# google/compare_gan

Hardware: NVIDIA H100
Metric: images/sec G+D step (resnet_cifar10) (higher is better)
Workload: dtype tf32

## Files before the change

### compare_gan_b200/_lib.py

```python
import ctypes
import os
import re

HERE = os.path.dirname(os.path.abspath(__file__))
HEADER = os.path.join(HERE, "..", "include", "cgan_b200.h")
SO_PATH = os.path.join(HERE, "csrc", "libcgan_b200.so")


class ConvDesc(ctypes.Structure):
  _fields_ = [(n, ctypes.c_int32) for n in
              ("n", "h", "w", "cin", "cout", "kh", "kw", "stride", "upsample", "oh", "ow", "pad_t", "pad_l")]


class ConvEpilogue(ctypes.Structure):
  _fields_ = [("bias", ctypes.c_void_p), ("residual", ctypes.c_void_p), ("mask", ctypes.c_void_p),
              ("mask_leak", ctypes.c_float), ("flags", ctypes.c_int32), ("ldy", ctypes.c_int32)]


CONV_RELU, CONV_ROUND_OUT, CONV_IN_TF32, CONV_IN2_TF32 = 1, 2, 4, 8
ACT_ROUND_TF32 = 0x100
OPT_TC_MT, OPT_LAST_PATH, OPT_TC_HALO, OPT_TC_THIN = 1, 2, 3, 6
OPT_LAST_TC_BN, OPT_LAST_TC_MT, OPT_LAST_TC_HALO, OPT_LAST_TC_CTAS_PER_SM = 7, 8, 9, 10
PATH_NAMES = {0: "simt_fp32", 1: "tcgen05_tf32", 2: "thin_fp32"}

_SCALARS = {"int": ctypes.c_int, "int32_t": ctypes.c_int32, "int64_t": ctypes.c_int64,
            "float": ctypes.c_float, "double": ctypes.c_double, "size_t": ctypes.c_size_t, "uint64_t": ctypes.c_uint64}


def parse_header(path=HEADER):
  src = open(path).read()
  src = re.sub(r"/\*.*?\*/", " ", src, flags=re.S)
  src = re.sub(r"//[^\n]*", " ", src)
  protos = {}
  for m in re.finditer(r"(const\s+char\s*\*|int64_t|int)\s+(cgan_\w+)\s*\(([^;{]*)\)\s*;", src):
    ret, name, args = m.group(1), m.group(2), m.group(3)
    restype = ctypes.c_char_p if "char" in ret else (ctypes.c_int64 if ret == "int64_t" else ctypes.c_int)
    argtypes = []
    args = args.strip()
    if args and args != "void":
      for a in args.split(","):
        a = a.strip()
        if "*" in a:
          argtypes.append(ctypes.c_void_p)
        else:
          ty = a.replace("const", "").split()[0]
          argtypes.append(_SCALARS[ty])
    protos[name] = (restype, argtypes)
  return protos


class CganError(RuntimeError):
  pass


_DLL = {}
# ... 65 lines not shown
```

### compare_gan_b200/csrc/common.cuh

```cuda
#pragma once
#include <cuda_runtime.h>
#include <stdint.h>
#include <stdio.h>
#include <string.h>

#include "../../include/cgan_b200.h"

struct cgan_ctx {
  int device;
  cudaStream_t stream;
  void* ws;
  size_t ws_bytes;
  int math_mode;
  int64_t launches;
  int num_sms;
  int tc_mt_max;
  int tc_halo;
  int tc_thin;
  int last_path;
  int last_tc_bn, last_tc_mt, last_tc_halo;
  int last_tc_ctas_per_sm;
  unsigned* counters;
  void* p2p;
  char err[512];
};

constexpr int CGAN_NUM_COUNTERS = 1 << 18;

static inline int cgan_fail(cgan_ctx* ctx, int code, const char* fmt, const char* a = "", const char* b = "") {
  if (ctx) snprintf(ctx->err, sizeof(ctx->err), fmt, a, b);
  return code;
}

#define CGAN_REQUIRE(ctx, cond, msg)                                              \
  do {                                                                            \
    if (!(cond)) return cgan_fail((ctx), CGAN_ERR_ARG, "%s: %s", __func__, msg);  \
  } while (0)

#define CGAN_CUDA(ctx, call)                                                                        \
  do {                                                                                              \
    cudaError_t e__ = (call);                                                                       \
    if (e__ != cudaSuccess) return cgan_fail((ctx), CGAN_ERR_CUDA, "%s: %s", __func__, cudaGetErrorString(e__)); \
  } while (0)

#define CGAN_LAUNCHED(ctx)                                                                          \
  do {                                                                                              \
    (ctx)->launches++;                                                                              \
    cudaError_t e__ = cudaGetLastError();                                                           \
    if (e__ != cudaSuccess) return cgan_fail((ctx), CGAN_ERR_CUDA, "%s: launch: %s", __func__, cudaGetErrorString(e__)); \
  } while (0)

static inline int cgan_ws(cgan_ctx* ctx, size_t bytes, void** out) {
  if (bytes > ctx->ws_bytes) {
    cudaStreamCaptureStatus st = cudaStreamCaptureStatusNone;
// ... 218 lines not shown
```

### compare_gan_b200/csrc/conv_tc.cu

```cuda
#include "tc_common.cuh"

namespace {

using namespace tc;

constexpr int TC_BM = 128;
constexpr int TC_BK = 32;
constexpr int TC_MAX_STAGES = 4;
constexpr int TC_MAX_TAPS = 32;
constexpr int TC_CWARPS = 8;
constexpr int TC_THREADS = 32 * TC_CWARPS + 32;
constexpr int TC_A_BYTES = TC_BM * TC_BK * 4;
constexpr int TC_WG_A_BYTES = TC_A_BYTES / 2;
constexpr int TC_ACC_COLS = 256;

struct TcParams {
  int ntaps, kchunks;
  int off_h[TC_MAX_TAPS], off_w[TC_MAX_TAPS], wtap[TC_MAX_TAPS], amap[TC_MAX_TAPS];
  int bw, bh, bni;
  int tiles_w, tiles_h;
  int rows_used;
  int img_n, img_h, img_w;
  int relu;
  int vec2;
  int round_a;
  int round_out;
  float mask_leak;
  const float* residual;
  const float* mask;
  int wimg_stride;
  int bn;
  int stages;
  int mt;
  int tiles_total;
  int cout;
  long long s_n, s_h, s_w, base;
  float* out;
  const float* bias;
  int nphases;
  int ph_tap0[5];
  long long ph_base[4];
  int hg, hnv;
  int h_off_w[4], h_off_h0[4], h_wtap[4][4];
  int a_halo_bytes;
  int a_box_bytes;
  int sa_stages, sb_stages;
};

struct AMaps { CUtensorMap m[4]; };


__device__ __forceinline__ void tc_tile_origin(const TcParams& p, int t, int& ow0, int& oh0, int& n0) {
  const int tw = t % p.tiles_w; t /= p.tiles_w;
  const int th = t % p.tiles_h;
  const int tn = t / p.tiles_h;
  ow0 = tw * p.bw; oh0 = th * p.bh; n0 = tn * p.bni;
}

__device__ __forceinline__ float epilogue_one(const TcParams& p, float v, int col, long long off) {
  if (p.bias) v += p.bias[col];
  if (p.residual) v += p.residual[off];
  if (p.relu) v = fmaxf(v, 0.f);
  if (p.mask) v = p.mask[off] > 0.f ? v : p.mask_leak * v;
  if (p.round_out) v = rna_tf32(v);
  return v;
}

template <int BN>
__device__ __forceinline__ void tile_epilogue(const TcParams& p, const float* acc, int tile, int nb0, int wg, int warp, int lane,
                                            long long out_base) {
  int ow0, oh0, n0;
  tc_tile_origin(p, tile, ow0, oh0, n0);
  const int c2 = (lane & 3) * 2;
#pragma unroll
  for (int h = 0; h < 2; ++h) {
    const int m = wg * 64 + (warp & 3) * 16 + (lane >> 2) + h * 8;
    const int wi = m % p.bw;
    const int hi = (m / p.bw) % p.bh;
    const int ni = m / (p.bw * p.bh);
    if (!(m < p.rows_used && n0 + ni < p.img_n && oh0 + hi < p.img_h && ow0 + wi < p.img_w)) continue;
    const long long roff = out_base + (long long)(n0 + ni) * p.s_n + (long long)(oh0 + hi) * p.s_h +
                           (long long)(ow0 + wi) * p.s_w + nb0;
#pragma unroll
    for (int j = 0; j < BN / 8; ++j) {
      const int c = j * 8 + c2;
      if (nb0 + c >= p.cout) continue;
      float2 v = make_float2(acc[4 * j + 2 * h], acc[4 * j + 2 * h + 1]);
      const long long off = roff + c;
      if (p.vec2) {
        if (p.bias) { const float2 b = *reinterpret_cast<const float2*>(p.bias + nb0 + c); v.x += b.x; v.y += b.y; }
        if (p.residual) { const float2 r = *reinterpret_cast<const float2*>(p.residual + off); v.x += r.x; v.y += r.y; }
        if (p.relu) { v.x = fmaxf(v.x, 0.f); v.y = fmaxf(v.y, 0.f); }
        if (p.mask) {
          const float2 mv = *reinterpret_cast<const float2*>(p.mask + off);
          v.x = mv.x > 0.f ? v.x : p.mask_leak * v.x; v.y = mv.y > 0.f ? v.y : p.mask_leak * v.y;
        }
        if (p.round_out) { v.x = rna_tf32(v.x); v.y = rna_tf32(v.y); }
        *reinterpret_cast<float2*>(p.out + off) = v;
      } else {
        p.out[off] = epilogue_one(p, v.x, nb0 + c, off);
        if (nb0 + c + 1 < p.cout) p.out[off + 1] = epilogue_one(p, v.y, nb0 + c + 1, off + 1);
      }
    }
  }
}

constexpr int tc_min_ctas(int bn, int mt) { return bn * mt <= 128 ? 2 : 1; }

__device__ __forceinline__ void tc_round_smem(uint32_t base, int bytes, int q, int nthreads) {
#pragma unroll 4
  for (int i = q * 16; i < bytes; i += nthreads * 16) {
    float4 v = lds128(base + i);
    v.x = rna_tf32(v.x); v.y = rna_tf32(v.y); v.z = rna_tf32(v.z); v.w = rna_tf32(v.w);
    sts128(base + i, v);
  }
}

template <int BN, int MT>
__global__ void __launch_bounds__(TC_THREADS, tc_min_ctas(BN, MT))
conv_tc_kernel(const __grid_constant__ AMaps tm_as, const __grid_constant__ CUtensorMap tm_b, const TcParams p) {
  extern __shared__ __align__(1024) uint8_t smem_raw[];
  uint8_t* smem = reinterpret_cast<uint8_t*>((reinterpret_cast<uintptr_t>(smem_raw) + 1023) & ~uintptr_t(1023));
  constexpr int b_bytes = BN * TC_BK * 4;
  constexpr int a_bytes = MT * TC_A_BYTES;
  constexpr int stage_bytes = a_bytes + b_bytes;
  uint64_t* full_bar = reinterpret_cast<uint64_t*>(smem + p.stages * stage_bytes);
  uint64_t* empty_bar = full_bar + p.stages;

  const int warp = threadIdx.x >> 5, lane = threadIdx.x & 31;
  const int tap0 = p.ph_tap0[blockIdx.z];
  const int num_kb = (p.ph_tap0[blockIdx.z + 1] - tap0) * p.kchunks;

  const int tile0 = blockIdx.x * MT;
  const int nt_here = max(0, min(MT, p.tiles_total - tile0));
  const int nb0 = blockIdx.y * BN;

  if (threadIdx.x == 0) {
    for (int s = 0; s < p.stages; ++s) {
      mbar_init(&full_bar[s], 1);
      mbar_init(&empty_bar[s], 2);
    }
    asm volatile("fence.mbarrier_init.release.cluster;" ::: "memory");
  }
  __syncthreads();

  if (warp == TC_CWARPS) {
    if (lane == 0) {
      asm volatile("prefetch.tensormap [%0];" ::"l"(&tm_as.m[0]) : "memory");
      asm volatile("prefetch.tensormap [%0];" ::"l"(&tm_b) : "memory");
      int stage = 0;
      uint32_t phase = 0;
      for (int kb = 0; kb < num_kb; ++kb) {
        const int tl = kb / p.kchunks, kc = kb - tl * p.kchunks, tap = tap0 + tl;
        mbar_wait(&empty_bar[stage], phase ^ 1);
        uint8_t* sa = smem + stage * stage_bytes;
        uint8_t* sb = sa + a_bytes;
        mbar_expect_tx(&full_bar[stage], (uint32_t)(nt_here * p.rows_used * TC_BK * 4 + b_bytes));
        int ow0, oh0, n0;
        for (int i = 0; i < nt_here; ++i) {
          tc_tile_origin(p, tile0 + i, ow0, oh0, n0);
          tma_load_4d(sa + i * TC_A_BYTES, &tm_as.m[p.amap[tap]], &full_bar[stage], kc * TC_BK, ow0 + p.off_w[tap],
                      oh0 + p.off_h[tap], n0);
        }
        tc_tile_origin(p, tile0, ow0, oh0, n0);
        tma_load_3d(sb, &tm_b, &full_bar[stage], kc * TC_BK, nb0, p.wtap[tap] + n0 * p.wimg_stride);
        if (++stage == p.stages) { stage = 0; phase ^= 1; }
      }
    }
  } else {
    const int wg = warp >> 2;
    const int q = threadIdx.x & 127;
    float acc[MT][BN / 2];
#pragma unroll
    for (int t = 0; t < MT; ++t)
#pragma unroll
      for (int i = 0; i < BN / 2; ++i) acc[t][i] = 0.f;
    int stage = 0, prev = -1;
    uint32_t phase = 0;
    for (int kb = 0; kb < num_kb; ++kb) {
      mbar_wait(&full_bar[stage], phase);
      const uint32_t a_addr = smem_u32(smem + stage * stage_bytes) + wg * TC_WG_A_BYTES;
      const uint32_t b_addr = smem_u32(smem + stage * stage_bytes) + a_bytes;
      if (p.round_a) {
        for (int tl = 0; tl < nt_here; ++tl) tc_round_smem(a_addr + tl * TC_A_BYTES, TC_WG_A_BYTES, q, 128);
        fence_proxy_async();
        named_bar(1 + wg, 128);
      }
#pragma unroll
      for (int t = 0; t < MT; ++t)
#pragma unroll
        for (int i = 0; i < BN / 2; ++i) acc_fence(acc[t][i]);
      wgmma_fence();
#pragma unroll
      for (int t = 0; t < MT; ++t) {
#pragma unroll
        for (int k = 0; k < TC_BK / 8; ++k)
          wgmma_tf32<BN>(acc[t], make_desc(a_addr + t * TC_A_BYTES + k * 32), make_desc(b_addr + k * 32));
      }
      wgmma_commit();
      wgmma_wait<1>();
#pragma unroll
      for (int t = 0; t < MT; ++t)
#pragma unroll
        for (int i = 0; i < BN / 2; ++i) acc_fence(acc[t][i]);
      if (prev >= 0 && q == 0) mbar_arrive(&empty_bar[prev]);
      prev = stage;
      if (++stage == p.stages) { stage = 0; phase ^= 1; }
    }
    wgmma_wait<0>();
#pragma unroll
    for (int t = 0; t < MT; ++t) {
#pragma unroll
      for (int i = 0; i < BN / 2; ++i) acc_fence(acc[t][i]);
      if (t < nt_here) tile_epilogue<BN>(p, acc[t], tile0 + t, nb0, wg, warp, lane, p.ph_base[blockIdx.z]);
    }
  }
}

template <int BN, int MT>
__global__ void __launch_bounds__(TC_THREADS, 1)
conv_tc_halo_kernel(const __grid_constant__ CUtensorMap tm_a, const __grid_constant__ CUtensorMap tm_b, const TcParams p) {
  extern __shared__ __align__(1024) uint8_t smem_raw[];
  uint8_t* smem = reinterpret_cast<uint8_t*>((reinterpret_cast<uintptr_t>(smem_raw) + 1023) & ~uintptr_t(1023));
  constexpr int b_bytes = BN * TC_BK * 4;
  const int a_stage = MT * p.a_halo_bytes;
  uint8_t* smem_b = smem + p.sa_stages * a_stage;
  uint64_t* a_full = reinterpret_cast<uint64_t*>(smem_b + p.sb_stages * b_bytes);
  uint64_t* a_empty = a_full + p.sa_stages;
  uint64_t* b_full = a_empty + p.sa_stages;
  uint64_t* b_empty = b_full + p.sb_stages;

  const int warp = threadIdx.x >> 5, lane = threadIdx.x & 31;
  const int tile0 = blockIdx.x * MT;
  const int nt_here = min(MT, p.tiles_total - tile0);
  const int nb0 = blockIdx.y * BN;

  if (threadIdx.x == 0) {
    for (int s = 0; s < p.sa_stages; ++s) {
      mbar_init(&a_full[s], 1);
      mbar_init(&a_empty[s], 2);
    }
    for (int s = 0; s < p.sb_stages; ++s) {
      mbar_init(&b_full[s], 1);
      mbar_init(&b_empty[s], 2);
    }
    asm volatile("fence.mbarrier_init.release.cluster;" ::: "memory");
  }
// ... 125 lines not shown
  int best = tc_pick_bn(ncols_pad);
  if (best == 0 || tiles_m * (ncols_pad / best) >= sms) return best;
  int pick = best;
  for (int b = best - 32; b >= 64; b -= 32) {
    if (ncols_pad % b) continue;
    pick = b;
    if (tiles_m * (ncols_pad / b) >= sms) break;
  }
  return pick;
}

constexpr int TC_NARROW_WAVES = 2;
constexpr int TC_NARROW_MAX_KB = 96;

inline int tc_pick_bn_per_tap(int ncols_pad, long long tiles_m, const TcParams& p, int sms) {
  const int bn = tc_pick_bn_occupancy(ncols_pad, tiles_m, sms);
  int kb = 0;
  for (int i = 0; i < p.nphases; ++i) {
    const int k = (p.ph_tap0[i + 1] - p.ph_tap0[i]) * p.kchunks;
    if (k > kb) kb = k;
  }
  if (bn == 256 && tiles_m * (ncols_pad / 256) * p.nphases >= (long long)TC_NARROW_WAVES * sms && kb <= TC_NARROW_MAX_KB)
    return 128;
  return bn;
}


inline int tc_vec2(const TcParams& p) {
  long long odd = p.cout | p.s_n | p.s_h | p.s_w | p.base;
  for (int i = 0; i < p.nphases; ++i) odd |= p.ph_base[i];
  return (odd & 1) ? 0 : 1;
}

int prep_weights(cgan_ctx* ctx, const TcConv& c, int kdim_pad, int ncols_pad, float** out) {
  void* ws = nullptr;
  int rc = cgan_ws(ctx, (size_t)c.taps_total * ncols_pad * kdim_pad * sizeof(float), &ws);
  if (rc) return rc;
  float* wt = reinterpret_cast<float*>(ws);
  long long tot = (long long)c.taps_total * ncols_pad * kdim_pad;
  long long blocks = (tot + 255) / 256, cap = (long long)ctx->num_sms * 8;
  wprep_kernel<<<(int)(blocks > cap ? cap : blocks), 256, 0, ctx->stream>>>(wt, c.wsrc, c.taps_total, c.ncols, ncols_pad, c.a.ch,
                                                                             kdim_pad, c.transpose_w);
  CGAN_LAUNCHED(ctx);
  *out = wt;
  return CGAN_OK;
}

bool make_weight_map(CUtensorMap* tm, float* wt, int kdim_pad, int ncols_pad, int taps_total, int bn) {
  cuuint64_t dims[3] = {(cuuint64_t)kdim_pad, (cuuint64_t)ncols_pad, (cuuint64_t)taps_total};
  cuuint64_t strides[2] = {(cuuint64_t)kdim_pad * 4, (cuuint64_t)ncols_pad * kdim_pad * 4};
  cuuint32_t box[3] = {TC_BK, (cuuint32_t)bn, 1};
  cuuint32_t es[3] = {1, 1, 1};
  return get_encode()(tm, CU_TENSOR_MAP_DATA_TYPE_FLOAT32, 3, wt, dims, strides, box, es, CU_TENSOR_MAP_INTERLEAVE_NONE,
                      CU_TENSOR_MAP_SWIZZLE_128B, CU_TENSOR_MAP_L2_PROMOTION_L2_256B,
                      CU_TENSOR_MAP_FLOAT_OOB_FILL_NONE) == CUDA_SUCCESS;
}

template <typename Kernel>
int tc_ctas_per_sm(Kernel kernel, size_t smem) {
  int blocks = 0;
  if (cudaOccupancyMaxActiveBlocksPerMultiprocessor(&blocks, kernel, TC_THREADS, smem) != cudaSuccess) blocks = 0;
  return blocks;
}

template <int BN, int MT>
int tc_launch_t(cgan_ctx* ctx, bool halo, dim3 grid, size_t smem, const AMaps& as, const CUtensorMap& b, const TcParams& p) {
  static bool attr_set[2] = {false, false};
  if (halo) {
    if (!attr_set[1]) {
      CGAN_CUDA(ctx, cudaFuncSetAttribute(conv_tc_halo_kernel<BN, MT>, cudaFuncAttributeMaxDynamicSharedMemorySize, 227 * 1024));
      attr_set[1] = true;
    }
    ctx->last_tc_ctas_per_sm = tc_ctas_per_sm(conv_tc_halo_kernel<BN, MT>, smem);
    conv_tc_halo_kernel<BN, MT><<<grid, TC_THREADS, smem, ctx->stream>>>(as.m[0], b, p);
  } else {
    if (!attr_set[0]) {
      CGAN_CUDA(ctx, cudaFuncSetAttribute(conv_tc_kernel<BN, MT>, cudaFuncAttributeMaxDynamicSharedMemorySize, 227 * 1024));
      attr_set[0] = true;
    }
    ctx->last_tc_ctas_per_sm = tc_ctas_per_sm(conv_tc_kernel<BN, MT>, smem);
    conv_tc_kernel<BN, MT><<<grid, TC_THREADS, smem, ctx->stream>>>(as, b, p);
  }
  CGAN_LAUNCHED(ctx);
  return CGAN_OK;
}

int tc_launch(cgan_ctx* ctx, bool halo, dim3 grid, size_t smem, const AMaps& as, const CUtensorMap& b, const TcParams& p) {
  ctx->last_tc_bn = p.bn; ctx->last_tc_mt = p.mt; ctx->last_tc_halo = halo ? 1 : 0;
#define TC_CASE(BN, MT) \
  if (p.bn == BN && p.mt == MT) return tc_launch_t<BN, MT>(ctx, halo, grid, smem, as, b, p);
  TC_CASE(32, 1) TC_CASE(64, 1) TC_CASE(96, 1) TC_CASE(128, 1) TC_CASE(160, 1) TC_CASE(192, 1) TC_CASE(224, 1)
  TC_CASE(256, 1) TC_CASE(32, 2) TC_CASE(64, 2) TC_CASE(96, 2) TC_CASE(128, 2)
#undef TC_CASE
  return cgan_fail(ctx, CGAN_ERR_UNSUPPORTED, "%s: no kernel for this column tile / pixel-tile count%s", "cgan_conv_tc");
}

}

bool cgan_tc_shape_ok(int n, int h, int w, int kdim, int ncols) {
  if (n < 1 || h < 1 || w < 1 || ncols < 1) return false;
  if (kdim < 8 || kdim % 4 != 0) return false;
  if (ncols > 256 && ncols % 32 != 0) return false;
  int bn = tc_pick_bn((ncols + 31) / 32 * 32);
  return bn != 0 && bn % 32 == 0;
}

int cgan_conv_tc(cgan_ctx* ctx, const TcConv& c) {
  if (!get_encode()) return cgan_fail(ctx, CGAN_ERR_UNSUPPORTED, "%s: cuTensorMapEncodeTiled unavailable%s", "cgan_conv_tc");
  const ConvTaps& tp = c.taps;
  if (tp.ntaps > TC_MAX_TAPS || c.a.nviews > 4) return cgan_fail(ctx, CGAN_ERR_UNSUPPORTED, "%s: too many taps/views%s", "cgan_conv_tc");
  const int n = c.a.n, h = c.a.h, w = c.a.w, kdim = c.a.ch, gh = c.gh, gw = c.gw, ntaps = tp.ntaps;
  TcParams p;
  memset(&p, 0, sizeof(p));
  p.ntaps = ntaps;
  const int kdim_pad = (kdim + TC_BK - 1) / TC_BK * TC_BK;
  p.kchunks = kdim_pad / TC_BK;
  for (int i = 0; i < ntaps; ++i) {
    p.off_h[i] = tp.off_h[i]; p.off_w[i] = tp.off_w[i]; p.wtap[i] = tp.wtap[i]; p.amap[i] = tp.view[i];
  }
  int tiles_n;
  tc_geometry(n, gh, gw, &p.bw, &p.bh, &p.bni, &p.tiles_w, &p.tiles_h, &tiles_n);
  p.rows_used = p.bw * p.bh * p.bni;
  p.img_n = n; p.img_h = gh; p.img_w = gw;
// ... 59 lines not shown
      p.tiles_w = w / hbw; p.tiles_h = h / hbh;
      const long long tiles_total = (long long)p.tiles_w * p.tiles_h * n;
      p.rows_used = 128;
      p.bn = tc_pick_bn_occupancy(ncols_pad, tiles_total, ctx->num_sms);
      const int ncol_tiles = ncols_pad / p.bn;
      p.a_box_bytes = (hbh + 2) * hbw * 128;
      p.a_halo_bytes = (p.a_box_bytes + 1023) / 1024 * 1024;
      const int b_bytes = p.bn * TC_BK * 4;
      const int budget = 227 * 1024 - 1024 - 512;
      const int mt_cap = ctx->tc_mt_max >= 2 ? 2 : 1;
      p.sa_stages = 2;
      p.mt = 1;
      for (int m = mt_cap; m >= 2; --m) {
        if (m * p.bn > TC_ACC_COLS || tiles_total * ncol_tiles < 2ll * m * ctx->num_sms) continue;
        if ((budget - p.sa_stages * m * p.a_halo_bytes) / b_bytes < 4) continue;
        p.mt = m;
        break;
      }
      p.sb_stages = (budget - p.sa_stages * p.mt * p.a_halo_bytes) / b_bytes;
      if (p.sb_stages > 8) p.sb_stages = 8;
      ok = p.sb_stages >= 2;
      if (ok) {
        p.tiles_total = (int)tiles_total;
        AMaps tm_a;
        CUtensorMap tm_b;
        memset(&tm_a, 0, sizeof(tm_a));
        if (!make_act_map(&tm_a.m[0], c.a.in + c.a.view_off[0], kdim, w, h, n, c.a.sw, c.a.sh, c.a.sn, hbw, hbh + 2, 1))
          return cgan_fail(ctx, CGAN_ERR_CUDA, "%s: cuTensorMapEncodeTiled(A halo) failed%s", "cgan_conv_tc");
        if (!make_weight_map(&tm_b, wt, kdim_pad, ncols_pad, c.taps_total, p.bn))
          return cgan_fail(ctx, CGAN_ERR_CUDA, "%s: cuTensorMapEncodeTiled(B) failed%s", "cgan_conv_tc");
        p.vec2 = tc_vec2(p);
        size_t smem = (size_t)p.sa_stages * p.mt * p.a_halo_bytes + (size_t)p.sb_stages * b_bytes + 1024 + 512;
        dim3 grid((unsigned)((tiles_total + p.mt - 1) / p.mt), (unsigned)ncol_tiles);
        return tc_launch(ctx, true, grid, smem, tm_a, tm_b, p);
      }
    }
    tc_geometry(n, gh, gw, &p.bw, &p.bh, &p.bni, &p.tiles_w, &p.tiles_h, &tiles_n);
    p.rows_used = p.bw * p.bh * p.bni;
    p.bn = tc_pick_bn_per_tap(ncols_pad, (long long)p.tiles_w * p.tiles_h * tiles_n, p, ctx->num_sms);
    p.hg = p.hnv = 0;
  }

  AMaps tm_as;
  CUtensorMap tm_b;
  memset(&tm_as, 0, sizeof(tm_as));
  for (int v = 0; v < 4; ++v)
    if (!make_view_map(&tm_as.m[v], c.a, v, p.bw, p.bh, p.bni))
      return cgan_fail(ctx, CGAN_ERR_CUDA, "%s: cuTensorMapEncodeTiled(A) failed%s", "cgan_conv_tc");
  if (!make_weight_map(&tm_b, wt, kdim_pad, ncols_pad, c.taps_total, p.bn))
    return cgan_fail(ctx, CGAN_ERR_CUDA, "%s: cuTensorMapEncodeTiled(B) failed%s", "cgan_conv_tc");

  const long long tiles_total = (long long)p.tiles_w * p.tiles_h * tiles_n;
  const int ncol_tiles = ncols_pad / p.bn;
  p.tiles_total = (int)tiles_total;
  p.mt = 1;
  if (ctx->tc_mt_max >= 2 && 2 * p.bn <= 128 && tiles_total * ncol_tiles * p.nphases >= 4ll * ctx->num_sms &&
      (c.wimg_stride == 0 || (p.tiles_w * p.tiles_h) % 2 == 0))
    p.mt = 2;
  const bool two_ctas = p.mt * p.bn <= 128;
  const size_t stage_bytes = (size_t)p.mt * TC_A_BYTES + (size_t)p.bn * TC_BK * 4;
  p.stages = (int)(((two_ctas ? 110 : 220) * 1024) / stage_bytes);
  if (p.stages > TC_MAX_STAGES) p.stages = TC_MAX_STAGES;
  if (p.stages < 2) p.stages = 2;
  p.vec2 = tc_vec2(p);
  size_t smem = (size_t)p.stages * stage_bytes + 1024  + 256 ;
  dim3 grid((unsigned)((tiles_total + p.mt - 1) / p.mt), (unsigned)ncol_tiles, (unsigned)p.nphases);
  return tc_launch(ctx, false, grid, smem, tm_as, tm_b, p);
}
```

### compare_gan_b200/csrc/pointwise.cu

```cuda
#include "common.cuh"

int cgan_version(void) { return 1; }

int cgan_ctx_create(cgan_ctx** out, int device) {
  if (!out) return CGAN_ERR_ARG;
  *out = nullptr;
  int count = 0;
  if (cudaGetDeviceCount(&count) != cudaSuccess || device < 0 || device >= count) return CGAN_ERR_CUDA;
  cgan_ctx* c = new cgan_ctx();
  memset(c, 0, sizeof(*c));
  c->device = device;
  if (cudaSetDevice(device) != cudaSuccess) { delete c; return CGAN_ERR_CUDA; }
  cudaDeviceProp prop;
  if (cudaGetDeviceProperties(&prop, device) != cudaSuccess) { delete c; return CGAN_ERR_CUDA; }
  c->num_sms = prop.multiProcessorCount;
  c->tc_mt_max = 2;
  if (const char* e = getenv("CGAN_TC_MT")) c->tc_mt_max = atoi(e) >= 2 ? 2 : 1;
  c->tc_halo = 1;
  if (const char* e = getenv("CGAN_TC_HALO")) c->tc_halo = atoi(e) ? 1 : 0;
  c->tc_thin = 1;
  if (const char* e = getenv("CGAN_TC_THIN")) c->tc_thin = atoi(e) ? 1 : 0;
  c->stream = 0;
  if (cudaMalloc(reinterpret_cast<void**>(&c->counters), CGAN_NUM_COUNTERS * sizeof(unsigned)) != cudaSuccess ||
      cudaMemset(c->counters, 0, CGAN_NUM_COUNTERS * sizeof(unsigned)) != cudaSuccess) {
// ... 33 lines not shown

int cgan_ctx_set_option(cgan_ctx* ctx, int key, int64_t value) {
  if (!ctx) return CGAN_ERR_ARG;
  switch (key) {
    case CGAN_OPT_TC_MT:
      CGAN_REQUIRE(ctx, value == 1 || value == 2, "CGAN_OPT_TC_MT must be 1 or 2");
      ctx->tc_mt_max = (int)value;
      return CGAN_OK;
    case CGAN_OPT_TC_HALO:
      CGAN_REQUIRE(ctx, value >= 0 && value <= 2, "CGAN_OPT_TC_HALO must be 0, 1 or 2");
      ctx->tc_halo = (int)value;
      return CGAN_OK;
    case CGAN_OPT_TC_THIN:
      CGAN_REQUIRE(ctx, value == 0 || value == 1, "CGAN_OPT_TC_THIN must be 0 or 1");
      ctx->tc_thin = (int)value;
      return CGAN_OK;
    default:
      return cgan_fail(ctx, CGAN_ERR_ARG, "%s: unknown or read-only option%s", "cgan_ctx_set_option");
  }
}

int cgan_ctx_get_option(cgan_ctx* ctx, int key, int64_t* host_value) {
  if (!ctx) return CGAN_ERR_ARG;
  CGAN_REQUIRE(ctx, host_value, "null pointer");
  switch (key) {
    case CGAN_OPT_TC_MT: *host_value = ctx->tc_mt_max; return CGAN_OK;
    case CGAN_OPT_LAST_PATH: *host_value = ctx->last_path; return CGAN_OK;
    case CGAN_OPT_TC_HALO: *host_value = ctx->tc_halo; return CGAN_OK;
    case CGAN_OPT_TC_THIN: *host_value = ctx->tc_thin; return CGAN_OK;
    case CGAN_OPT_LAST_TC_BN: *host_value = ctx->last_tc_bn; return CGAN_OK;
    case CGAN_OPT_LAST_TC_MT: *host_value = ctx->last_tc_mt; return CGAN_OK;
    case CGAN_OPT_LAST_TC_HALO: *host_value = ctx->last_tc_halo; return CGAN_OK;
    case CGAN_OPT_LAST_TC_CTAS_PER_SM: *host_value = ctx->last_tc_ctas_per_sm; return CGAN_OK;
    default:
      return cgan_fail(ctx, CGAN_ERR_ARG, "%s: unknown option%s", "cgan_ctx_get_option");
  }
}

const char* cgan_last_error(cgan_ctx* ctx) { return ctx ? ctx->err : "null context"; }
int64_t cgan_launch_count(cgan_ctx* ctx) { return ctx ? ctx->launches : -1; }

namespace {

#define EW_LOOP(i, n)                                                                  \
  for (long long i = (long long)blockIdx.x * blockDim.x + threadIdx.x, s__ = (long long)gridDim.x * blockDim.x; \
       i < (n); i += s__)

__global__ void fill_kernel(float* d, float v, long long n) { EW_LOOP(i, n) d[i] = v; }
__global__ void copy_kernel(float* __restrict__ d, const float* __restrict__ s, long long n) { EW_LOOP(i, n) d[i] = s[i]; }
__global__ void copy2d_kernel(float* __restrict__ d, int dld, int doff, const float* __restrict__ s, int sld, int soff,
                              long long rows, int cols) {
  long long n = rows * cols;
  EW_LOOP(i, n) {
    long long r = i / cols;
    int j = (int)(i % cols);
    d[r * dld + doff + j] = s[r * sld + soff + j];
  }
}
__global__ void axpby_kernel(float* __restrict__ y, float a, const float* __restrict__ x, float b,
                             const float* __restrict__ y0, float c, long long n) {
  EW_LOOP(i, n) {
    float v = a * x[i] + c;
    if (y0) v += b * y0[i];
    y[i] = v;
  }
}
// ... 810 lines not shown
```

### compare_gan_b200/csrc/tc_common.cuh

```cuda
#pragma once
#include <cuda.h>

#include "common.cuh"
#include "wgmma_tf32.cuh"

namespace tc {

__device__ __forceinline__ uint32_t smem_u32(const void* p) { return (uint32_t)__cvta_generic_to_shared(p); }

__device__ __forceinline__ void mbar_init(uint64_t* bar, uint32_t count) {
  asm volatile("mbarrier.init.shared::cta.b64 [%0], %1;" ::"r"(smem_u32(bar)), "r"(count));
}
__device__ __forceinline__ void mbar_expect_tx(uint64_t* bar, uint32_t bytes) {
  asm volatile("mbarrier.arrive.expect_tx.shared::cta.b64 _, [%0], %1;" ::"r"(smem_u32(bar)), "r"(bytes) : "memory");
}
__device__ __forceinline__ void mbar_arrive(uint64_t* bar) {
  asm volatile("mbarrier.arrive.shared::cta.b64 _, [%0];" ::"r"(smem_u32(bar)) : "memory");
}
__device__ __forceinline__ void mbar_wait(uint64_t* bar, uint32_t parity) {
  uint32_t addr = smem_u32(bar);
  asm volatile(
      "{\n\t"
      ".reg .pred p;\n\t"
      "WAIT_LOOP:\n\t"
// ... 11 lines not shown
}
__device__ __forceinline__ void tma_load_3d(void* dst, const CUtensorMap* map, uint64_t* bar, int c0, int c1, int c2) {
  asm volatile(
      "cp.async.bulk.tensor.3d.shared::cluster.global.tile.mbarrier::complete_tx::bytes [%0], [%1, {%3, %4, %5}], [%2];"
      ::"r"(smem_u32(dst)), "l"(map), "r"(smem_u32(bar)), "r"(c0), "r"(c1), "r"(c2) : "memory");
}

__device__ __forceinline__ uint64_t make_desc(uint32_t smem_addr) {
  uint64_t d = 0;
  d |= (uint64_t)((smem_addr & 0x3FFFF) >> 4);
  d |= (uint64_t)1 << 16;
  d |= (uint64_t)(1024 >> 4) << 32;
  d |= (uint64_t)1 << 62;
  return d;
}

__device__ __forceinline__ void wgmma_fence() { asm volatile("wgmma.fence.sync.aligned;" ::: "memory"); }
__device__ __forceinline__ void wgmma_commit() { asm volatile("wgmma.commit_group.sync.aligned;" ::: "memory"); }
template <int N>
__device__ __forceinline__ void wgmma_wait() { asm volatile("wgmma.wait_group.sync.aligned %0;" ::"n"(N) : "memory"); }
__device__ __forceinline__ void acc_fence(float& r) { asm volatile("" : "+f"(r)::"memory"); }
__device__ __forceinline__ void named_bar(int id, int count) { asm volatile("bar.sync %0, %1;" ::"r"(id), "r"(count) : "memory"); }
__device__ __forceinline__ void fence_proxy_async() { asm volatile("fence.proxy.async.shared::cta;" ::: "memory"); }

__device__ __forceinline__ uint32_t sw128_offset(int row, int k) {
  return (uint32_t)(row * 128 + ((((k >> 2) ^ row) & 7) << 4) + (k & 3) * 4);
}

__device__ __forceinline__ float4 lds128(uint32_t addr) {
  float4 v;
  asm volatile("ld.shared.v4.f32 {%0, %1, %2, %3}, [%4];" : "=f"(v.x), "=f"(v.y), "=f"(v.z), "=f"(v.w) : "r"(addr));
  return v;
}
__device__ __forceinline__ float lds32(uint32_t addr) {
  float v;
  asm volatile("ld.shared.f32 %0, [%1];" : "=f"(v) : "r"(addr));
  return v;
}
__device__ __forceinline__ void sts128(uint32_t addr, float4 v) {
  asm volatile("st.shared.v4.f32 [%0], {%1, %2, %3, %4};" ::"r"(addr), "f"(v.x), "f"(v.y), "f"(v.z), "f"(v.w) : "memory");
}

typedef CUresult (*EncodeTiledFn)(CUtensorMap*, CUtensorMapDataType, cuuint32_t, void*, const cuuint64_t*, const cuuint64_t*,
                                  const cuuint32_t*, const cuuint32_t*, CUtensorMapInterleave, CUtensorMapSwizzle,
                                  CUtensorMapL2promotion, CUtensorMapFloatOOBfill);

inline EncodeTiledFn get_encode() {
  static EncodeTiledFn fn = nullptr;
  if (!fn) {
    void* p = nullptr;
    cudaDriverEntryPointQueryResult q;
    if (cudaGetDriverEntryPoint("cuTensorMapEncodeTiled", &p, cudaEnableDefault, &q) == cudaSuccess &&
        q == cudaDriverEntryPointSuccess)
      fn = reinterpret_cast<EncodeTiledFn>(p);
  }
  return fn;
}


inline bool make_act_map(CUtensorMap* tm, const float* base, int c, int w, int h, int n, long long sw, long long sh,
                         long long sn, int bw, int bh, int bni, CUtensorMapSwizzle swizzle = CU_TENSOR_MAP_SWIZZLE_128B) {
  EncodeTiledFn enc = get_encode();
  if (!enc) return false;
  cuuint64_t dims[4] = {(cuuint64_t)c, (cuuint64_t)w, (cuuint64_t)h, (cuuint64_t)n};
  cuuint64_t strides[3] = {(cuuint64_t)sw * 4, (cuuint64_t)sh * 4, (cuuint64_t)sn * 4};
  cuuint32_t box[4] = {32, (cuuint32_t)bw, (cuuint32_t)bh, (cuuint32_t)bni};
// ... 17 lines not shown
```

### include/cgan_b200.h

```cpp
#ifndef CGAN_B200_H_
#define CGAN_B200_H_

#include <stddef.h>
#include <stdint.h>

#ifdef __cplusplus
extern "C" {
#endif

typedef struct cgan_ctx cgan_ctx;

enum { CGAN_OK = 0, CGAN_ERR_ARG = 1, CGAN_ERR_CUDA = 2, CGAN_ERR_WORKSPACE = 3, CGAN_ERR_UNSUPPORTED = 4 };

int cgan_version(void);
int cgan_ctx_create(cgan_ctx** out, int device);
int cgan_ctx_destroy(cgan_ctx* ctx);
int cgan_ctx_set_stream(cgan_ctx* ctx, void* cuda_stream);
int cgan_ctx_reserve_workspace(cgan_ctx* ctx, size_t bytes);
int cgan_ctx_set_math_mode(cgan_ctx* ctx, int mode);
const char* cgan_last_error(cgan_ctx* ctx);
int64_t cgan_launch_count(cgan_ctx* ctx);
enum { CGAN_OPT_TC_MT = 1, CGAN_OPT_LAST_PATH = 2, CGAN_OPT_TC_HALO = 3, CGAN_OPT_TC_THIN = 6, CGAN_OPT_LAST_TC_BN = 7,
       CGAN_OPT_LAST_TC_MT = 8, CGAN_OPT_LAST_TC_HALO = 9, CGAN_OPT_LAST_TC_CTAS_PER_SM = 10 };
enum { CGAN_PATH_SIMT_FP32 = 0, CGAN_PATH_TCGEN05_TF32 = 1, CGAN_PATH_THIN_FP32 = 2 };
int cgan_ctx_set_option(cgan_ctx* ctx, int key, int64_t value);
int cgan_ctx_get_option(cgan_ctx* ctx, int key, int64_t* host_value);

int cgan_fill(cgan_ctx*, float* dst, float value, int64_t n);
int cgan_copy(cgan_ctx*, float* dst, const float* src, int64_t n);
int cgan_copy2d(cgan_ctx*, float* dst, int dst_ld, int dst_off, const float* src, int src_ld, int src_off,
                int64_t rows, int cols);
int cgan_axpby(cgan_ctx*, float* y, float a, const float* x, float b, const float* y0, float c, int64_t n);
int cgan_scale_by_dev(cgan_ctx*, float* y, const float* x, const float* scalar_dev, float mul, int inverse, int64_t n);
int cgan_dot(cgan_ctx*, float* out_dev, const float* a, const float* b, int64_t n);
int cgan_random_uniform(cgan_ctx*, float* out, int64_t n, uint64_t seed, uint64_t offset);
int cgan_interpolate(cgan_ctx*, float* y, const float* x, const float* xf, const float* alpha, int n, int64_t per);
int cgan_one_hot(cgan_ctx*, float* out, const int32_t* labels, int n, int classes);

typedef struct {
  int32_t n, h, w, cin;
  int32_t cout, kh, kw, stride;
  int32_t upsample;
  int32_t oh, ow;
  int32_t pad_t, pad_l;
} cgan_conv_desc;

int cgan_conv2d_fwd(cgan_ctx*, const cgan_conv_desc*, const float* x, const float* w_hwio, const float* bias, float* y);
int cgan_conv2d_fwd_act(cgan_ctx*, const cgan_conv_desc*, const float* x, const float* w_hwio, const float* bias, int act,
                        float* y);
int cgan_conv2d_fwd_act_ld(cgan_ctx*, const cgan_conv_desc*, const float* x, const float* w_hwio, const float* bias, int act,
                           float* y, int ldy);
int cgan_conv2d_dgrad(cgan_ctx*, const cgan_conv_desc*, const float* dy, const float* w_hwio, float* dx);
int cgan_conv2d_wgrad(cgan_ctx*, const cgan_conv_desc*, const float* x, const float* dy, float* dw);
enum { CGAN_CONV_RELU = 1, CGAN_CONV_ROUND_OUT = 2, CGAN_CONV_IN_TF32 = 4, CGAN_CONV_IN2_TF32 = 8 };
typedef struct {
  const float* bias;
// ... 149 lines not shown
```

### profiles/tile_ab.py

```python
import argparse
import hashlib
import json
import os
import statistics
import subprocess
import sys

TF32_PEAK_TFLOPS = 495.0

SHAPES = [
    ("cifar G up 3x3 256->256 4->8", 256, 4, 256, 256, 3, True),
    ("cifar G up 3x3 256->256 8->16", 256, 8, 256, 256, 3, True),
    ("cifar G up 3x3 256->256 16->32", 256, 16, 256, 256, 3, True),
    ("cifar G 3x3 256->256 @8", 256, 8, 256, 256, 3, False),
    ("cifar G 3x3 256->256 @16", 256, 16, 256, 256, 3, False),
    ("cifar G 3x3 256->256 @32", 256, 32, 256, 256, 3, False),
    ("cifar G up 1x1 256->256 4->8", 256, 4, 256, 256, 1, True),
    ("cifar G up 1x1 256->256 8->16", 256, 8, 256, 256, 1, True),
    ("cifar G up 1x1 256->256 16->32", 256, 16, 256, 256, 1, True),
    ("cifar D 3x3 128->128 @32", 512, 32, 128, 128, 3, False),
    ("cifar D 1x1 128->128 @32", 512, 32, 128, 128, 1, False),
    ("cifar D 3x3 128->128 @16", 512, 16, 128, 128, 3, False),
    ("cifar D 3x3 128->128 @8", 512, 8, 128, 128, 3, False),
    ("biggan G up 3x3 1536->1536 4->8", 64, 4, 1536, 1536, 3, True),
# ... 23 lines not shown
    torch.cuda.synchronize()
    st = torch.cuda.current_stream()
    e0, e1 = torch.cuda.Event(enable_timing=True), torch.cuda.Event(enable_timing=True)
    e0.record(st)
    for _ in range(iters):
      fn()
    e1.record(st)
    torch.cuda.synchronize()
    return e0.elapsed_time(e1) / iters

  def rand(*shape):
    return K.from_numpy((np.random.RandomState(sum(shape)).standard_normal(shape) * 0.1).astype(np.float32))

  K.init(0)
  K.set_math_mode(1)
  lib = K.lib()
  ctas_key = getattr(_lib, "OPT_LAST_TC_CTAS_PER_SM", None)

  def digest(t):
    return hashlib.sha1(np.ascontiguousarray(t.cpu()).tobytes()).hexdigest()[:12]

  def geometry():
    g = "bn%d mt%d%s" % (lib.get_option(_lib.OPT_LAST_TC_BN), lib.get_option(_lib.OPT_LAST_TC_MT),
                         " halo" if lib.get_option(_lib.OPT_LAST_TC_HALO) else "")
    if ctas_key is not None:
      g += " %d/SM" % lib.get_option(ctas_key)
    return g

  rows = []
  for label, b, h, cin, cout, k, up in SHAPES:
    x, w, bias = rand(b, h, h, cin), rand(k, k, cin, cout), K.zeros(cout)
    d = K.conv_desc(b, h, h, cin, cout, k, k, 1, up, "SAME")
    dy = rand(b, d.oh, d.ow, cout)
    taps = k * k / 4.0 if up else k * k
    flop = 2.0 * b * d.oh * d.ow * taps * cin * cout
    with tape.no_record():
      for pre in (False, True):
        x.tf32 = dy.tf32 = K.tf32_on() if pre else False
        suffix = " pre" if pre else ""
        for op, fn in (("fwd", lambda: K.conv2d(x, w, bias, upsample=up)), ("dgrad", lambda: K.conv2d_dgrad(d, dy, w))):
          ms = timed(fn)
          rows.append({"shape": label, "op": op + suffix, "ms": ms, "gflop": flop / 1e9, "geometry": geometry(),
                       "digest": digest(fn())})
        for mt in (2, 1):
          lib.set_option(_lib.OPT_TC_MT, mt)
          fn = lambda: K.conv2d_wgrad(d, x, dy)
          ms = timed(fn)
          rows.append({"shape": label, "op": "wgrad%s" % suffix, "ms": ms, "gflop": flop / 1e9,
                       "geometry": "tc_mt %d" % mt, "digest": digest(fn())})
        lib.set_option(_lib.OPT_TC_MT, 2)
    del x, w, dy
    torch.cuda.empty_cache()
  print(json.dumps({"device": torch.cuda.get_device_name(0), "rows": rows}))


def card():
  try:
    return subprocess.run(["nvidia-smi", "--query-gpu=name,power.limit,clocks.sm,clocks.max.sm", "--format=csv,noheader"],
                          capture_output=True, text=True, timeout=30).stdout.strip()
  except (OSError, subprocess.SubprocessError) as e:
    return "nvidia-smi unavailable (%s)" % e


def main():
  ap = argparse.ArgumentParser()
  ap.add_argument("--tree", action="append", default=[], help="source tree with a built library (give two)")
  ap.add_argument("--rounds", type=int, default=3)
  ap.add_argument("--out", default="tile_ab_out")
  ap.add_argument("--child", help=argparse.SUPPRESS)
  args = ap.parse_args()
  if args.child:
    return child(args.child)
  if len(args.tree) != 2:
    raise SystemExit("give two --tree arguments")
  info = {"card_before": card(), "trees": args.tree, "rounds": args.rounds}
  runs = {t: [] for t in args.tree}
  for r in range(args.rounds):
    for t in args.tree:
      out = subprocess.run([sys.executable, os.path.abspath(__file__), "--child", t], capture_output=True, text=True)
      if out.returncode != 0:
        sys.stderr.write(out.stdout + out.stderr)
        raise SystemExit("child for %s failed" % t)
      runs[t].append(json.loads(out.stdout.strip().splitlines()[-1]))
  info["card_after"] = card()
  info["device"] = runs[args.tree[0]][0]["device"]
  table = []
  for i, row in enumerate(runs[args.tree[0]][0]["rows"]):
    entry = {"shape": row["shape"], "op": row["op"], "gflop": row["gflop"]}
    for j, t in enumerate(args.tree):
      ms = [run["rows"][i]["ms"] for run in runs[t]]
      key = "ab"[j]
      entry[key + "_geometry"] = runs[t][0]["rows"][i]["geometry"]
      entry[key + "_ms"] = statistics.median(ms)
      entry[key + "_spread"] = max(ms) - min(ms)
      entry[key + "_tf32_share"] = row["gflop"] / entry[key + "_ms"] / TF32_PEAK_TFLOPS
    entry["same_bits"] = len({run["rows"][i]["digest"] for t in args.tree for run in runs[t]}) == 1
    table.append(entry)
  print("%s | %s -> %s" % (info["device"], info["card_before"], info["card_after"]))
  print("A = %s, B = %s, median of %d rounds" % (args.tree[0], args.tree[1], args.rounds))
  print("%-34s %-10s %8s | %-28s %8s %6s | %-28s %8s %6s | %6s %s" % (
      "shape", "op", "GFLOP", "A geometry", "A ms", "A pk%", "B geometry", "B ms", "B pk%", "B/A", "bits"))
  for e in table:
    print("%-34s %-10s %8.1f | %-28s %8.3f %5.1f%% | %-28s %8.3f %5.1f%% | %6.3f %s" % (
        e["shape"], e["op"], e["gflop"], e["a_geometry"], e["a_ms"], 100 * e["a_tf32_share"], e["b_geometry"], e["b_ms"],
        100 * e["b_tf32_share"], e["b_ms"] / e["a_ms"], "same" if e["same_bits"] else "DIFFER"))
  os.makedirs(args.out, exist_ok=True)
  with open(os.path.join(args.out, "tile_ab.json"), "w") as f:
    json.dump({"info": info, "rows": table}, f, indent=1)


if __name__ == "__main__":
  main()
```

Baseline: 20230.

## Stage residual/mask epilogue operands through TMA into shared memory pipeline stages

When a conv has exactly one residual or mask operand with aligned strides, the producer warp issues TMA loads of that operand's tile into the freed pipeline stages after the main loop. The consumer warps read it from swizzled shared memory instead of doing scattered global loads in the epilogue. Bias is also cached in shared memory. This replaces uncoalesced per-thread global reads with bulk async copies, at the cost of extra barrier handshakes, extra shared memory, and more epilogue complexity.

New measurement: 21600, median of 6. 1.07x the previous value.

```diff
diff --git a/compare_gan_b200/_lib.py b/compare_gan_b200/_lib.py
--- a/compare_gan_b200/_lib.py
+++ b/compare_gan_b200/_lib.py
@@ -20,7 +20,7 @@
 CONV_RELU, CONV_ROUND_OUT, CONV_IN_TF32, CONV_IN2_TF32 = 1, 2, 4, 8
 ACT_ROUND_TF32 = 0x100
 OPT_TC_MT, OPT_LAST_PATH, OPT_TC_HALO, OPT_TC_THIN = 1, 2, 3, 6
-OPT_LAST_TC_BN, OPT_LAST_TC_MT, OPT_LAST_TC_HALO, OPT_LAST_TC_CTAS_PER_SM = 7, 8, 9, 10
+OPT_LAST_TC_BN, OPT_LAST_TC_MT, OPT_LAST_TC_HALO, OPT_LAST_TC_CTAS_PER_SM, OPT_LAST_TC_EP_SMEM = 7, 8, 9, 10, 11
 PATH_NAMES = {0: "simt_fp32", 1: "tcgen05_tf32", 2: "thin_fp32"}
 
 _SCALARS = {"int": ctypes.c_int, "int32_t": ctypes.c_int32, "int64_t": ctypes.c_int64,
diff --git a/compare_gan_b200/csrc/common.cuh b/compare_gan_b200/csrc/common.cuh
--- a/compare_gan_b200/csrc/common.cuh
+++ b/compare_gan_b200/csrc/common.cuh
@@ -20,6 +20,7 @@
   int last_path;
   int last_tc_bn, last_tc_mt, last_tc_halo;
   int last_tc_ctas_per_sm;
+  int last_tc_ep_smem;
   unsigned* counters;
   void* p2p;
   char err[512];
diff --git a/compare_gan_b200/csrc/conv_tc.cu b/compare_gan_b200/csrc/conv_tc.cu
--- a/compare_gan_b200/csrc/conv_tc.cu
+++ b/compare_gan_b200/csrc/conv_tc.cu
@@ -45,6 +45,7 @@
   int a_halo_bytes;
   int a_box_bytes;
   int sa_stages, sb_stages;
+  int ep_smem;
 };
 
 struct AMaps { CUtensorMap m[4]; };
@@ -105,6 +106,59 @@
   }
 }
 
+template <int BN>
+__device__ __forceinline__ void tile_epilogue_smem(const TcParams& p, const float* acc, int tile, int nb0, int wg, int warp,
+                                                 int lane, long long out_base, const uint8_t* smem, int stage_bytes,
+                                                 uint64_t* full_bar, uint64_t* empty_bar, int& stage, uint32_t& phase,
+                                                 int& chunk, int chunks, const float* s_bias) {
+  int ow0, oh0, n0;
+  tc_tile_origin(p, tile, ow0, oh0, n0);
+  const int c2 = (lane & 3) * 2;
+  bool ok[2];
+  long long roff[2];
+  int m[2];
+#pragma unroll
+  for (int h = 0; h < 2; ++h) {
+    m[h] = wg * 64 + (warp & 3) * 16 + (lane >> 2) + h * 8;
+    const int wi = m[h] % p.bw;
+    const int hi = (m[h] / p.bw) % p.bh;
+    const int ni = m[h] / (p.bw * p.bh);
+    ok[h] = m[h] < p.rows_used && n0 + ni < p.img_n && oh0 + hi < p.img_h && ow0 + wi < p.img_w;
+    roff[h] = out_base + (long long)(n0 + ni) * p.s_n + (long long)(oh0 + hi) * p.s_h + (long long)(ow0 + wi) * p.s_w + nb0;
+  }
+  const uint32_t bias_addr = smem_u32(s_bias);
+#pragma unroll
+  for (int cc = 0; cc < BN / 32; ++cc) {
+    mbar_wait(&full_bar[stage], phase);
+    const uint32_t e_addr = smem_u32(smem + stage * stage_bytes);
+#pragma unroll
+    for (int jj = 0; jj < 4; ++jj) {
+      const int j = cc * 4 + jj, c = j * 8 + c2;
+      if (nb0 + c >= p.cout) continue;
+      const float2 b = p.bias ? lds64(bias_addr + c * 4) : make_float2(0.f, 0.f);
+#pragma unroll
+      for (int h = 0; h < 2; ++h) {
+        if (!ok[h]) continue;
+        float2 v = make_float2(acc[4 * j + 2 * h], acc[4 * j + 2 * h + 1]);
+        const float2 e = lds64(e_addr + sw128_offset(m[h], jj * 8 + c2));
+        if (p.bias) { v.x += b.x; v.y += b.y; }
+        if (p.residual) { v.x += e.x; v.y += e.y; }
+        if (p.relu) { v.x = fmaxf(v.x, 0.f); v.y = fmaxf(v.y, 0.f); }
+        if (p.mask) { v.x = e.x > 0.f ? v.x : p.mask_leak * v.x; v.y = e.y > 0.f ? v.y : p.mask_leak * v.y; }
+        if (p.round_out) { v.x = rna_tf32(v.x); v.y = rna_tf32(v.y); }
+        *reinterpret_cast<float2*>(p.out + roff[h] + c) = v;
+      }
+    }
+    if (chunk + p.stages < chunks) {
+      fence_proxy_async();
+      named_bar(1 + wg, 128);
+      if ((threadIdx.x & 127) == 0) mbar_arrive(&empty_bar[stage]);
+    }
+    ++chunk;
+    if (++stage == p.stages) { stage = 0; phase ^= 1; }
+  }
+}
+
 constexpr int tc_min_ctas(int bn, int mt) { return bn * mt <= 128 ? 2 : 1; }
 
 __device__ __forceinline__ void tc_round_smem(uint32_t base, int bytes, int q, int nthreads) {
@@ -118,7 +172,8 @@
 
 template <int BN, int MT>
 __global__ void __launch_bounds__(TC_THREADS, tc_min_ctas(BN, MT))
-conv_tc_kernel(const __grid_constant__ AMaps tm_as, const __grid_constant__ CUtensorMap tm_b, const TcParams p) {
+conv_tc_kernel(const __grid_constant__ AMaps tm_as, const __grid_constant__ CUtensorMap tm_b, const TcParams p,
+               const __grid_constant__ AMaps tm_e) {
   extern __shared__ __align__(1024) uint8_t smem_raw[];
   uint8_t* smem = reinterpret_cast<uint8_t*>((reinterpret_cast<uintptr_t>(smem_raw) + 1023) & ~uintptr_t(1023));
   constexpr int b_bytes = BN * TC_BK * 4;
@@ -126,6 +181,7 @@
   constexpr int stage_bytes = a_bytes + b_bytes;
   uint64_t* full_bar = reinterpret_cast<uint64_t*>(smem + p.stages * stage_bytes);
   uint64_t* empty_bar = full_bar + p.stages;
+  float* s_bias = reinterpret_cast<float*>(smem + p.stages * stage_bytes + 256);
 
   const int warp = threadIdx.x >> 5, lane = threadIdx.x & 31;
   const int tap0 = p.ph_tap0[blockIdx.z];
@@ -166,10 +222,25 @@
         tma_load_3d(sb, &tm_b, &full_bar[stage], kc * TC_BK, nb0, p.wtap[tap] + n0 * p.wimg_stride);
         if (++stage == p.stages) { stage = 0; phase ^= 1; }
       }
+      if (p.ep_smem) {
+        const CUtensorMap* em = &tm_e.m[blockIdx.z];
+        for (int t = 0; t < nt_here; ++t) {
+          int ow0, oh0, n0;
+          tc_tile_origin(p, tile0 + t, ow0, oh0, n0);
+          for (int cc = 0; cc < BN / 32; ++cc) {
+            mbar_wait(&empty_bar[stage], phase ^ 1);
+            mbar_expect_tx(&full_bar[stage], (uint32_t)(p.rows_used * TC_BK * 4));
+            tma_load_4d(smem + stage * stage_bytes, em, &full_bar[stage], nb0 + cc * 32, ow0, oh0, n0);
+            if (++stage == p.stages) { stage = 0; phase ^= 1; }
+          }
+        }
+      }
     }
   } else {
     const int wg = warp >> 2;
     const int q = threadIdx.x & 127;
+    if (p.ep_smem && p.bias)
+      for (int i = threadIdx.x; i < BN; i += 32 * TC_CWARPS) s_bias[i] = nb0 + i < p.cout ? p.bias[nb0 + i] : 0.f;
     float acc[MT][BN / 2];
 #pragma unroll
     for (int t = 0; t < MT; ++t)
@@ -208,11 +279,25 @@
       if (++stage == p.stages) { stage = 0; phase ^= 1; }
     }
     wgmma_wait<0>();
-#pragma unroll
-    for (int t = 0; t < MT; ++t) {
-#pragma unroll
-      for (int i = 0; i < BN / 2; ++i) acc_fence(acc[t][i]);
-      if (t < nt_here) tile_epilogue<BN>(p, acc[t], tile0 + t, nb0, wg, warp, lane, p.ph_base[blockIdx.z]);
+    if (p.ep_smem) {
+      if (prev >= 0 && q == 0) mbar_arrive(&empty_bar[prev]);
+      named_bar(3, 32 * TC_CWARPS);
+      int chunk = 0;
+#pragma unroll
+      for (int t = 0; t < MT; ++t) {
+#pragma unroll
+        for (int i = 0; i < BN / 2; ++i) acc_fence(acc[t][i]);
+        if (t < nt_here)
+          tile_epilogue_smem<BN>(p, acc[t], tile0 + t, nb0, wg, warp, lane, p.ph_base[blockIdx.z], smem, stage_bytes,
+                                 full_bar, empty_bar, stage, phase, chunk, nt_here * (BN / 32), s_bias);
+      }
+    } else {
+#pragma unroll
+      for (int t = 0; t < MT; ++t) {
+#pragma unroll
+        for (int i = 0; i < BN / 2; ++i) acc_fence(acc[t][i]);
+        if (t < nt_here) tile_epilogue<BN>(p, acc[t], tile0 + t, nb0, wg, warp, lane, p.ph_base[blockIdx.z]);
+      }
     }
   }
 }
@@ -404,6 +489,14 @@
   return (odd & 1) ? 0 : 1;
 }
 
+inline bool tc_ep_smem_ok(const TcParams& p, const TcConv& c) {
+  const float* e = c.residual ? c.residual : c.mask;
+  if (!e || (c.residual && c.mask) || !p.vec2 || (reinterpret_cast<uintptr_t>(e) & 15)) return false;
+  long long a = p.s_n | p.s_h | p.s_w;
+  for (int i = 0; i < p.nphases; ++i) a |= p.ph_base[i];
+  return (a & 3) == 0;
+}
+
 int prep_weights(cgan_ctx* ctx, const TcConv& c, int kdim_pad, int ncols_pad, float** out) {
   void* ws = nullptr;
   int rc = cgan_ws(ctx, (size_t)c.taps_total * ncols_pad * kdim_pad * sizeof(float), &ws);
@@ -436,7 +529,8 @@
 }
 
 template <int BN, int MT>
-int tc_launch_t(cgan_ctx* ctx, bool halo, dim3 grid, size_t smem, const AMaps& as, const CUtensorMap& b, const TcParams& p) {
+int tc_launch_t(cgan_ctx* ctx, bool halo, dim3 grid, size_t smem, const AMaps& as, const CUtensorMap& b, const TcParams& p,
+                const AMaps& es) {
   static bool attr_set[2] = {false, false};
   if (halo) {
     if (!attr_set[1]) {
@@ -451,16 +545,17 @@
       attr_set[0] = true;
     }
     ctx->last_tc_ctas_per_sm = tc_ctas_per_sm(conv_tc_kernel<BN, MT>, smem);
-    conv_tc_kernel<BN, MT><<<grid, TC_THREADS, smem, ctx->stream>>>(as, b, p);
+    conv_tc_kernel<BN, MT><<<grid, TC_THREADS, smem, ctx->stream>>>(as, b, p, es);
   }
   CGAN_LAUNCHED(ctx);
   return CGAN_OK;
 }
 
-int tc_launch(cgan_ctx* ctx, bool halo, dim3 grid, size_t smem, const AMaps& as, const CUtensorMap& b, const TcParams& p) {
-  ctx->last_tc_bn = p.bn; ctx->last_tc_mt = p.mt; ctx->last_tc_halo = halo ? 1 : 0;
+int tc_launch(cgan_ctx* ctx, bool halo, dim3 grid, size_t smem, const AMaps& as, const CUtensorMap& b, const TcParams& p,
+              const AMaps& es) {
+  ctx->last_tc_bn = p.bn; ctx->last_tc_mt = p.mt; ctx->last_tc_halo = halo ? 1 : 0; ctx->last_tc_ep_smem = p.ep_smem;
 #define TC_CASE(BN, MT) \
-  if (p.bn == BN && p.mt == MT) return tc_launch_t<BN, MT>(ctx, halo, grid, smem, as, b, p);
+  if (p.bn == BN && p.mt == MT) return tc_launch_t<BN, MT>(ctx, halo, grid, smem, as, b, p, es);
   TC_CASE(32, 1) TC_CASE(64, 1) TC_CASE(96, 1) TC_CASE(128, 1) TC_CASE(160, 1) TC_CASE(192, 1) TC_CASE(224, 1)
   TC_CASE(256, 1) TC_CASE(32, 2) TC_CASE(64, 2) TC_CASE(96, 2) TC_CASE(128, 2)
 #undef TC_CASE
@@ -586,7 +681,7 @@
         p.vec2 = tc_vec2(p);
         size_t smem = (size_t)p.sa_stages * p.mt * p.a_halo_bytes + (size_t)p.sb_stages * b_bytes + 1024 + 512;
         dim3 grid((unsigned)((tiles_total + p.mt - 1) / p.mt), (unsigned)ncol_tiles);
-        return tc_launch(ctx, true, grid, smem, tm_a, tm_b, p);
+        return tc_launch(ctx, true, grid, smem, tm_a, tm_b, p, tm_a);
       }
     }
     tc_geometry(n, gh, gw, &p.bw, &p.bh, &p.bni, &p.tiles_w, &p.tiles_h, &tiles_n);
@@ -617,7 +712,14 @@
   if (p.stages > TC_MAX_STAGES) p.stages = TC_MAX_STAGES;
   if (p.stages < 2) p.stages = 2;
   p.vec2 = tc_vec2(p);
-  size_t smem = (size_t)p.stages * stage_bytes + 1024  + 256 ;
+  AMaps tm_e;
+  memset(&tm_e, 0, sizeof(tm_e));
+  p.ep_smem = tc_ep_smem_ok(p, c) ? 1 : 0;
+  for (int v = 0; p.ep_smem && v < p.nphases; ++v)
+    if (!make_act_map(&tm_e.m[v], (c.residual ? c.residual : c.mask) + p.ph_base[v], c.ncols, gw, gh, n, p.s_w, p.s_h,
+                      p.s_n, p.bw, p.bh, p.bni))
+      return cgan_fail(ctx, CGAN_ERR_CUDA, "%s: cuTensorMapEncodeTiled(residual / mask) failed%s", "cgan_conv_tc");
+  size_t smem = (size_t)p.stages * stage_bytes + 1024  + 256  + (p.ep_smem ? p.bn * 4 : 0) ;
   dim3 grid((unsigned)((tiles_total + p.mt - 1) / p.mt), (unsigned)ncol_tiles, (unsigned)p.nphases);
-  return tc_launch(ctx, false, grid, smem, tm_as, tm_b, p);
-}
+  return tc_launch(ctx, false, grid, smem, tm_as, tm_b, p, tm_e);
+}
diff --git a/compare_gan_b200/csrc/pointwise.cu b/compare_gan_b200/csrc/pointwise.cu
--- a/compare_gan_b200/csrc/pointwise.cu
+++ b/compare_gan_b200/csrc/pointwise.cu
@@ -89,6 +89,7 @@
     case CGAN_OPT_LAST_TC_MT: *host_value = ctx->last_tc_mt; return CGAN_OK;
     case CGAN_OPT_LAST_TC_HALO: *host_value = ctx->last_tc_halo; return CGAN_OK;
     case CGAN_OPT_LAST_TC_CTAS_PER_SM: *host_value = ctx->last_tc_ctas_per_sm; return CGAN_OK;
+    case CGAN_OPT_LAST_TC_EP_SMEM: *host_value = ctx->last_tc_ep_smem; return CGAN_OK;
     default:
       return cgan_fail(ctx, CGAN_ERR_ARG, "%s: unknown option%s", "cgan_ctx_get_option");
   }
diff --git a/compare_gan_b200/csrc/tc_common.cuh b/compare_gan_b200/csrc/tc_common.cuh
--- a/compare_gan_b200/csrc/tc_common.cuh
+++ b/compare_gan_b200/csrc/tc_common.cuh
@@ -67,6 +67,11 @@
   asm volatile("ld.shared.v4.f32 {%0, %1, %2, %3}, [%4];" : "=f"(v.x), "=f"(v.y), "=f"(v.z), "=f"(v.w) : "r"(addr));
   return v;
 }
+__device__ __forceinline__ float2 lds64(uint32_t addr) {
+  float2 v;
+  asm volatile("ld.shared.v2.f32 {%0, %1}, [%2];" : "=f"(v.x), "=f"(v.y) : "r"(addr));
+  return v;
+}
 __device__ __forceinline__ float lds32(uint32_t addr) {
   float v;
   asm volatile("ld.shared.f32 %0, [%1];" : "=f"(v) : "r"(addr));
diff --git a/include/cgan_b200.h b/include/cgan_b200.h
--- a/include/cgan_b200.h
+++ b/include/cgan_b200.h
@@ -21,7 +21,8 @@
 const char* cgan_last_error(cgan_ctx* ctx);
 int64_t cgan_launch_count(cgan_ctx* ctx);
 enum { CGAN_OPT_TC_MT = 1, CGAN_OPT_LAST_PATH = 2, CGAN_OPT_TC_HALO = 3, CGAN_OPT_TC_THIN = 6, CGAN_OPT_LAST_TC_BN = 7,
-       CGAN_OPT_LAST_TC_MT = 8, CGAN_OPT_LAST_TC_HALO = 9, CGAN_OPT_LAST_TC_CTAS_PER_SM = 10 };
+       CGAN_OPT_LAST_TC_MT = 8, CGAN_OPT_LAST_TC_HALO = 9, CGAN_OPT_LAST_TC_CTAS_PER_SM = 10,
+       CGAN_OPT_LAST_TC_EP_SMEM = 11 };
 enum { CGAN_PATH_SIMT_FP32 = 0, CGAN_PATH_TCGEN05_TF32 = 1, CGAN_PATH_THIN_FP32 = 2 };
 int cgan_ctx_set_option(cgan_ctx* ctx, int key, int64_t value);
 int cgan_ctx_get_option(cgan_ctx* ctx, int key, int64_t* host_value);
diff --git a/profiles/tile_ab.py b/profiles/tile_ab.py
--- a/profiles/tile_ab.py
+++ b/profiles/tile_ab.py
@@ -79,13 +79,20 @@
     x, w, bias = rand(b, h, h, cin), rand(k, k, cin, cout), K.zeros(cout)
     d = K.conv_desc(b, h, h, cin, cout, k, k, 1, up, "SAME")
     dy = rand(b, d.oh, d.ow, cout)
+    ep_bias = rand(cout)
+    res = None if up else rand(b, d.oh, d.ow, cout)
+    mask = (rand(b, h, h, cin), 0.0)
     taps = k * k / 4.0 if up else k * k
     flop = 2.0 * b * d.oh * d.ow * taps * cin * cout
     with tape.no_record():
       for pre in (False, True):
         x.tf32 = dy.tf32 = K.tf32_on() if pre else False
         suffix = " pre" if pre else ""
-        for op, fn in (("fwd", lambda: K.conv2d(x, w, bias, upsample=up)), ("dgrad", lambda: K.conv2d_dgrad(d, dy, w))):
+        ops = [("fwd", lambda: K.conv2d(x, w, bias, upsample=up)), ("dgrad", lambda: K.conv2d_dgrad(d, dy, w))]
+        if res is not None:
+          ops.append(("fwd+res", lambda: K.conv2d(x, w, ep_bias, upsample=up, residual=res)))
+        ops.append(("dgrad+mask", lambda: K.conv2d_dgrad(d, dy, w, round_out=True, relu_mask=mask)))
+        for op, fn in ops:
           ms = timed(fn)
           rows.append({"shape": label, "op": op + suffix, "ms": ms, "gflop": flop / 1e9, "geometry": geometry(),
                        "digest": digest(fn())})
@@ -96,7 +103,7 @@
           rows.append({"shape": label, "op": "wgrad%s" % suffix, "ms": ms, "gflop": flop / 1e9,
                        "geometry": "tc_mt %d" % mt, "digest": digest(fn())})
         lib.set_option(_lib.OPT_TC_MT, 2)
-    del x, w, dy
+    del x, w, dy, res, mask
     torch.cuda.empty_cache()
   print(json.dumps({"device": torch.cuda.get_device_name(0), "rows": rows}))
 
@@ -143,14 +150,25 @@
       entry[key + "_tf32_share"] = row["gflop"] / entry[key + "_ms"] / TF32_PEAK_TFLOPS
     entry["same_bits"] = len({run["rows"][i]["digest"] for t in args.tree for run in runs[t]}) == 1
     table.append(entry)
+  bare = {(e["shape"], e["op"]): e for e in table}
+  for e in table:
+    if "+" in e["op"]:
+      op, _, rest = e["op"].partition("+")
+      pre = " pre" if rest.endswith(" pre") else ""
+      b = bare[(e["shape"], op + pre)]
+      for key in "ab":
+        e[key + "_gap"] = e[key + "_ms"] - b[key + "_ms"]
   print("%s | %s -> %s" % (info["device"], info["card_before"], info["card_after"]))
   print("A = %s, B = %s, median of %d rounds" % (args.tree[0], args.tree[1], args.rounds))
-  print("%-34s %-10s %8s | %-28s %8s %6s | %-28s %8s %6s | %6s %s" % (
-      "shape", "op", "GFLOP", "A geometry", "A ms", "A pk%", "B geometry", "B ms", "B pk%", "B/A", "bits"))
+  print("%-34s %-15s %8s | %-28s %8s %6s %7s | %-28s %8s %6s %7s | %6s %s" % (
+      "shape", "op", "GFLOP", "A geometry", "A ms", "A pk%", "A gap", "B geometry", "B ms", "B pk%", "B gap", "B/A",
+      "bits"))
+  gap = lambda e, key: "%7.3f" % e[key + "_gap"] if key + "_gap" in e else "%7s" % "-"
   for e in table:
-    print("%-34s %-10s %8.1f | %-28s %8.3f %5.1f%% | %-28s %8.3f %5.1f%% | %6.3f %s" % (
-        e["shape"], e["op"], e["gflop"], e["a_geometry"], e["a_ms"], 100 * e["a_tf32_share"], e["b_geometry"], e["b_ms"],
-        100 * e["b_tf32_share"], e["b_ms"] / e["a_ms"], "same" if e["same_bits"] else "DIFFER"))
+    print("%-34s %-15s %8.1f | %-28s %8.3f %5.1f%% %s | %-28s %8.3f %5.1f%% %s | %6.3f %s" % (
+        e["shape"], e["op"], e["gflop"], e["a_geometry"], e["a_ms"], 100 * e["a_tf32_share"], gap(e, "a"),
+        e["b_geometry"], e["b_ms"], 100 * e["b_tf32_share"], gap(e, "b"), e["b_ms"] / e["a_ms"],
+        "same" if e["same_bits"] else "DIFFER"))
   os.makedirs(args.out, exist_ok=True)
   with open(os.path.join(args.out, "tile_ab.json"), "w") as f:
     json.dump({"info": info, "rows": table}, f, indent=1)
```
